# Siverteh/semantic-slam-master

Measured on AMD Instinct MI355X. Metric: frames/sec extract+match on TUM 640x480; match-index bit-exact vs CPU ref, higher is better.
Workload: dtype f32

## Files before the change

semantic-slam-master_amd/csrc/common.h:

```cpp
#pragma once

#include <hip/hip_runtime.h>
#include <stdint.h>

#include "../../include/sslam_hip.h"

typedef float f32x16 __attribute__((ext_vector_type(16)));
typedef float f32x4 __attribute__((ext_vector_type(4)));

extern long long g_sslam_launches;
static inline void sslam_count_launches(long long n) { __atomic_fetch_add(&g_sslam_launches, n, __ATOMIC_RELAXED); }

enum sslam_knob_id {
    KNOB_M1_VARIANT,
    KNOB_CONV_VARIANT,
    KNOB_CONV_LATENCY_ROWS,
    KNOB_CONV_LAT2_ROWS,
    KNOB_CONV_NO_HALO,
    KNOB_CONV_TAIL,
    KNOB_CONVBF_NO_HALO,
    KNOB_CONVBF_TAIL,
    KNOB_CONVBF_VARIANT,
    KNOB_VIT_NO_FUSED_MLP,
    KNOB_BN_FORM,
    KNOB_VIT_F32_NO_KEY_SPLIT,
    KNOB_RT_STOP,
    KNOB_REFINE_DISTINCT,
    KNOB_COUNT
};
#define SSLAM_KNOB_UNSET (-0x7fffffffffffffffLL - 1)
extern long long g_sslam_knob[KNOB_COUNT];
static inline long long sslam_knob(int id, long long dflt) { const long long v = g_sslam_knob[id]; return v == SSLAM_KNOB_UNSET ? dflt : v; }
static inline bool sslam_knob_set(int id) { return g_sslam_knob[id] != SSLAM_KNOB_UNSET; }

template <class... P>
static inline bool sslam_misaligned(unsigned a, P... p) {
    uintptr_t bits = 0;
    const uintptr_t each[] = {(uintptr_t)p...};
    for (const uintptr_t v : each) bits |= v;
    return (bits & (uintptr_t)(a - 1)) != 0;
}

#define SSLAM_CHECK_LAUNCH()                                   \
    do {                                                       \
        sslam_count_launches(1);                               \
        if (hipGetLastError() != hipSuccess) return SSLAM_E_LAUNCH; \
    } while (0)

__host__ __device__ inline int kp8(int k) { return (k & ~7) | ((k & 1) << 2) | ((k & 7) >> 1); }

__device__ __forceinline__ f32x16 mfma32(float a, float b, f32x16 c) {
    return __builtin_amdgcn_mfma_f32_32x32x2f32(a, b, c, 0, 0, 0);
}

__device__ __forceinline__ int crow(int r, int h) { return (r & 3) + 8 * (r >> 2) + 4 * h; }

__device__ __forceinline__ float bfly32(float v) {
    v = v + __shfl_xor(v, 16);
    v = v + __shfl_xor(v, 8);
    v = v + __shfl_xor(v, 4);
// ... 52 lines not shown
```

semantic-slam-master_amd/csrc/lib.hip:

```cpp
#include <stdlib.h>
#include <string.h>

#include "common.h"

long long g_sslam_launches = 0;
long long g_sslam_knob[KNOB_COUNT];

namespace {
long long g_knob_at_load[KNOB_COUNT];
const char *const kKnobNames[KNOB_COUNT] = {
    "SSLAM_M1_VARIANT",   "SSLAM_CONV_VARIANT",  "SSLAM_CONV_LATENCY_ROWS", "SSLAM_CONV_LAT2_ROWS",   "SSLAM_CONV_NO_HALO",
    "SSLAM_CONV_TAIL",    "SSLAM_CONVBF_NO_HALO", "SSLAM_CONVBF_TAIL",      "SSLAM_CONVBF_VARIANT",   "SSLAM_VIT_NO_FUSED_MLP",
    "SSLAM_BN_FORM",      "SSLAM_VIT_F32_NO_KEY_SPLIT", "SSLAM_RT_STOP",
    "SSLAM_REFINE_DISTINCT"};
struct KnobInit {
    KnobInit() {
        for (int i = 0; i < KNOB_COUNT; i++) {
            const char *e = getenv(kKnobNames[i]);
            g_sslam_knob[i] = g_knob_at_load[i] = e ? atoll(e) : SSLAM_KNOB_UNSET;
        }
    }
} g_knob_init;
}

extern "C" int sslam_version(void) { return 650; }
extern "C" const char *sslam_arch(void) { return "gfx950"; }
extern "C" long long sslam_launch_count(void) { return __atomic_load_n(&g_sslam_launches, __ATOMIC_RELAXED); }

extern "C" long long sslam_workspace_bytes(int n_frames, int G, int K, int n_pairs) {
    if (n_frames <= 0 || G <= 0 || K <= 0 || n_pairs < 0) return SSLAM_E_INVALID;
    const long long a = sslam_selector_saliency_workspace_bytes(n_frames, G);
    const long long b = n_pairs > 0 ? sslam_sim_argmax_workspace_bytes(K, n_pairs) : 0;
    const long long c = sslam_gather_refine_workspace_bytes(n_frames, K);
    const long long m = a > b ? (a > c ? a : c) : (b > c ? b : c);
    return (m + 255) & ~255LL;
}

extern "C" int sslam_test_set_knob(const char *name, long long value, int unset) {
    if (!name) return SSLAM_E_INVALID;
    for (int i = 0; i < KNOB_COUNT; i++)
        if (!strcmp(name, kKnobNames[i])) {
            g_sslam_knob[i] = unset ? g_knob_at_load[i] : value;
            return SSLAM_OK;
        }
    return SSLAM_E_INVALID;
}
```

semantic-slam-master_amd/csrc/selector.hip:

```cpp
#include <stdlib.h>

#include "common.h"

namespace {

constexpr int BK = 32;
constexpr int LDT = BK + 4;
constexpr int NCHUNK = SSLAM_C / BK;
constexpr int NSTAGE = 9 * NCHUNK;

template <int WM, int WN, int NI, bool BDIRECT, int MI = 2>
__global__ __launch_bounds__(512, (BDIRECT && WM == 2) ? 4 : 1) void selector_saliency_kernel(const float *__restrict__ feat, int n_rows, int G,
                                                                 const float *__restrict__ w1p,
                                                                 const float *__restrict__ b1,
                                                                 const float *__restrict__ w2,
                                                                 const float *__restrict__ b2, float *__restrict__ sal,
                                                                 int n_tiles) {
    static_assert(WM * WN == 8, "8 waves");
    static_assert(MI == 2 || (MI == 1 && NI == 1 && BDIRECT), "latency form: one 32 x 32 tile per wave");
    constexpr int BM = 32 * MI * WM;
    constexpr int HS = 32 * NI * WN;
    constexpr int NSLAB = HS / 64;
    constexpr int A_ITEMS = BM * 4 >= 512 ? BM * 4 / 512 : 1;
    constexpr bool A_PART = BM * 4 < 512;
// ... 171 lines not shown
            for (int e = 0; e < 16; e++) {
                const float h1 = acc[0][0][e] > 0.0f ? acc[0][0][e] : 0.0f;
                xch[(slab * 16 + e) * 64 + lane] = h1 * w2v;
            }
        }
        __syncthreads();
        if (!(wn & 1)) {
#pragma unroll
            for (int e = 0; e < 16; e++) {
                const float h0 = acc[0][0][e] > 0.0f ? acc[0][0][e] : 0.0f;
                const float q = h0 * w2v + xch[(slab * 16 + e) * 64 + lane];
                const float t = bfly32(q);
                if (r == 0) red[slab * BM + crow(e, h)] = t;
            }
        }
    }
    __syncthreads();
    for (int t = tid; t < BM; t += 512) {
        const long long m = m0 + t;
        if (m < n_rows) {
            float logit = b2[0];
#pragma unroll
            for (int s = 0; s < NSLAB; s++) logit = logit + red[s * BM + t];
            sal[m] = sslam_sigmoid(logit);
        }
    }
}
#undef LOAD_STAGE
#undef STORE_STAGE

constexpr int HIMG_ROWS = 256;
constexpr int HIMG_FLOATS = HIMG_ROWS * LDT;

template <bool SMALL>
__device__ __forceinline__ void halo_tile(float *hsmem, const float *__restrict__ feat, int n_rows, int G, const float *__restrict__ w1p,
                                          const float *__restrict__ b1, const float *__restrict__ w2, const float *__restrict__ b2,
                                          float *__restrict__ sal, const int m0, const int m_end) {
    constexpr int WN = SMALL ? 8 : 4, NI = SMALL ? 1 : 2, MI = SMALL ? 1 : 2, BM = 32 * MI * (8 / WN), HS = 256, NSLAB = 4;
    const int tid = threadIdx.x, lane = tid & 63, wave = tid >> 6, r = lane & 31, h = lane >> 5;
    const int wm = wave / WN, wn = wave % WN;
    const int cells = G * G, G1 = G + 1, P = (G + 2) * G1;
    auto padded = [&](int m) {
        const int f = m / cells, c = m - f * cells, y = c / G, x = c - y * G;
        return f * P + (y + 1) * G1 + x;
    };
    const int p_lo = padded(m0) - (G + 2);

    const __amdgpu_buffer_rsrc_t frs =
        __builtin_amdgcn_make_buffer_rsrc(const_cast<float *>(feat), 0, (int)((unsigned)n_rows * (SSLAM_C * 4u)), 0x00020000);
    const int kq = tid & 3;
    int a_voff[2];
#pragma unroll
    for (int i = 0; i < 2; i++) {
        const int pr = p_lo + (tid >> 2) + 128 * i;
        int off = -32;
        if (pr >= 0) {
            const int f = pr / P, q = pr - f * P, yy = q / G1, xx = q - yy * G1;
            const long long m = (long long)f * cells + (yy - 1) * G + xx;
            if (yy >= 1 && yy <= G && xx < G && m < n_rows) off = (int)((unsigned)m * (SSLAM_C * 4u) + kq * 32u);
        }
        a_voff[i] = off;
    }
    float4 ra_lo, ra_hi;
#define HL(I, C)                                                                                                   \
    {                                                                                                              \
        ra_lo = __builtin_bit_cast(float4, __builtin_amdgcn_raw_buffer_load_b128(frs, a_voff[I], (C) * (BK * 4), 0));      \
        ra_hi = __builtin_bit_cast(float4, __builtin_amdgcn_raw_buffer_load_b128(frs, a_voff[I], (C) * (BK * 4) + 16, 0)); \
    }
#define HS_(I, BUF)                                                                                                \
    {                                                                                                              \
        float4 ev, od;                                                                                             \
        kp8_split(ra_lo, ra_hi, ev, od);                                                                           \
        float *d = hsmem + (BUF) * HIMG_FLOATS + ((tid >> 2) + 128 * (I)) * LDT + kq * 8;                          \
        *reinterpret_cast<float4 *>(d) = ev;                                                                       \
        *reinterpret_cast<float4 *>(d + 4) = od;                                                                   \
    }

    int a_base[MI];
#pragma unroll
    for (int mi = 0; mi < MI; mi++) {
        const int m = min(m0 + wm * 32 * MI + mi * 32 + r, m_end - 1);
        a_base[mi] = (padded(m) - p_lo) * LDT + 4 * h;
    }

    f32x16 acc[MI][NI];
#pragma unroll
    for (int ni = 0; ni < NI; ni++) {
        const float bv = b1[wn * 32 * NI + ni * 32 + r];
#pragma unroll
        for (int mi = 0; mi < MI; mi++)
#pragma unroll
            for (int e = 0; e < 16; e++) acc[mi][ni][e] = bv;
    }
    const f32x4 *bsrc = reinterpret_cast<const f32x4 *>(w1p) + ((wn * 32 * NI + r) * 2 + h);
    const __amdgpu_buffer_rsrc_t wrs =
        __builtin_amdgcn_make_buffer_rsrc(const_cast<float *>(w1p), 0, 9 * SSLAM_C * HS * 4, 0x00020000);
    const int b_voff = ((wn * 32 * NI + r) * 2 + h) * 16;
    f32x4 bq[BK / 8][NI];
#pragma unroll
    for (int g = 0; g < BK / 8; g++)
#pragma unroll
        for (int ni = 0; ni < NI; ni++) bq[g][ni] = bsrc[((long long)g * HS + ni * 32) * 2];

    HL(0, 0);
    HS_(0, 0);
    HL(1, 0);
    HS_(1, 0);
    __syncthreads();
    int tap = 0, dy = -1, dx = -1, chunk = 0;
    for (int s = 0; s < NSTAGE; s++) {
        if (chunk + 1 < NCHUNK) {
            if (tap == 0) HL(0, chunk + 1);
            if (tap == 4) {
                HS_(0, (chunk + 1) & 1);
                HL(1, chunk + 1);
            }
        }
        const float *img = hsmem + (chunk & 1) * HIMG_FLOATS + (dy * G1 + dx) * LDT;
        const float *A0 = img + a_base[0], *A1 = img + a_base[MI - 1];
        __builtin_amdgcn_s_setprio(1);
#pragma unroll
        for (int g = 0; g < BK / 8; g++) {
            const f32x4 a0 = *reinterpret_cast<const f32x4 *>(A0 + 8 * g);
            f32x4 a1 = a0;
            if (MI == 2) a1 = *reinterpret_cast<const f32x4 *>(A1 + 8 * g);
            f32x4 b[NI];
#pragma unroll
            for (int ni = 0; ni < NI; ni++) b[ni] = bq[g][ni];
#pragma unroll
            for (int st = 0; st < 4; st++)
#pragma unroll
                for (int ni = 0; ni < NI; ni++) {
                    acc[0][ni] = mfma32(a0[st], b[ni][st], acc[0][ni]);
                    if (MI == 2) acc[MI - 1][ni] = mfma32(a1[st], b[ni][st], acc[MI - 1][ni]);
                }
            if (s + 1 < NSTAGE && (g == BK / 16 - 1 || g == BK / 8 - 1)) {
#pragma unroll
                for (int gg = g + 1 - BK / 16; gg <= g; gg++)
#pragma unroll
                    for (int ni = 0; ni < NI; ni++)
                        bq[gg][ni] = __builtin_bit_cast(f32x4, __builtin_amdgcn_raw_buffer_load_b128(
                                                            wrs, b_voff, (((s + 1) * (BK / 8) + gg) * HS + ni * 32) * 32, 0));
            }
            if (g == BK / 16 - 1) __builtin_amdgcn_sched_barrier(0);
        }
        __builtin_amdgcn_s_setprio(0);
        tap++; dx++;
        if (dx == 2) { dx = -1; dy++; }
        if (tap == 9) {
            if (chunk + 1 < NCHUNK) HS_(1, (chunk + 1) & 1);
            __syncthreads();
            tap = 0; dy = -1; chunk++;
        }
    }
#undef HL
#undef HS_
    __syncthreads();
    float *red = hsmem;
    if (!SMALL) {
#pragma unroll
        for (int sl = 0; sl < NI / 2; sl++) {
            const int slab = wn * (NI / 2) + sl;
            const float w2a = w2[slab * 64 + r], w2b = w2[slab * 64 + 32 + r];
#pragma unroll
            for (int mi = 0; mi < MI; mi++)
#pragma unroll
                for (int e = 0; e < 16; e++) {
                    const float h0 = acc[mi][2 * sl][e] > 0.0f ? acc[mi][2 * sl][e] : 0.0f;
                    const float h1 = acc[mi][NI > 1 ? 2 * sl + 1 : 0][e] > 0.0f ? acc[mi][NI > 1 ? 2 * sl + 1 : 0][e] : 0.0f;
                    const float q = h0 * w2a + h1 * w2b;
                    const float t = bfly32(q);
                    if (r == 0) red[slab * BM + wm * 64 + mi * 32 + crow(e, h)] = t;
                }
        }
    } else {
        float *xch = hsmem + NSLAB * BM;
        const int slab = wn >> 1;
        const float w2v = w2[wn * 32 + r];
        if (wn & 1) {
#pragma unroll
            for (int e = 0; e < 16; e++) {
                const float h1 = acc[0][0][e] > 0.0f ? acc[0][0][e] : 0.0f;
                xch[(slab * 16 + e) * 64 + lane] = h1 * w2v;
            }
        }
        __syncthreads();
        if (!(wn & 1)) {
#pragma unroll
            for (int e = 0; e < 16; e++) {
                const float h0 = acc[0][0][e] > 0.0f ? acc[0][0][e] : 0.0f;
                const float q = h0 * w2v + xch[(slab * 16 + e) * 64 + lane];
                const float t = bfly32(q);
                if (r == 0) red[slab * BM + crow(e, h)] = t;
            }
        }
    }
    __syncthreads();
    for (int t = tid; t < BM; t += 512) {
        const long long m = (long long)m0 + t;
        if (m < m_end) {
            float logit = b2[0];
#pragma unroll
            for (int sb = 0; sb < NSLAB; sb++) logit = logit + red[sb * BM + t];
            sal[m] = sslam_sigmoid(logit);
        }
    }
}

__global__ __launch_bounds__(512, 4) void selector_saliency_halo_kernel(const float *__restrict__ feat, int n_rows, int G,
                                                                         const float *__restrict__ w1p, const float *__restrict__ b1,
                                                                         const float *__restrict__ w2, const float *__restrict__ b2,
                                                                         float *__restrict__ sal, int n_big) {
    extern __shared__ __attribute__((aligned(16))) float hsmem[];
    const int b = blockIdx.x;
    if (b < n_big) {
        const int q = n_big / 8, rem = n_big % 8, x = b % 8;
        const int tile = (x < rem ? x * (q + 1) : rem * (q + 1) + (x - rem) * q) + b / 8;
        halo_tile<false>(hsmem, feat, n_rows, G, w1p, b1, w2, b2, sal, tile * 128, n_rows);
    } else {
        halo_tile<true>(hsmem, feat, n_rows, G, w1p, b1, w2, b2, sal, n_big * 128 + (b - n_big) * 32, n_rows);
    }
}

__global__ __launch_bounds__(512, 4) void selector_saliency_halo_frames_kernel(const float *__restrict__ feat, int n_rows, int G,
                                                                                const float *__restrict__ w1p, const float *__restrict__ b1,
                                                                                const float *__restrict__ w2, const float *__restrict__ b2,
                                                                                float *__restrict__ sal, int n_big, int n_quarter, int tb, int ts) {
    extern __shared__ __attribute__((aligned(16))) float hsmem[];
    const int b = blockIdx.x, cells = G * G;
    if (b < n_big) {
        const int q = n_big / 8, rem = n_big % 8, x = b % 8;
        const int tile = (x < rem ? x * (q + 1) : rem * (q + 1) + (x - rem) * q) + b / 8;
        const int f = tile / tb, j = tile - f * tb;
        halo_tile<false>(hsmem, feat, n_rows, G, w1p, b1, w2, b2, sal, f * cells + j * 128, (f + 1) * cells);
    } else if (b < n_big + n_quarter) {
        const int u = b - n_big, tile = n_big + (u >> 2);
        const int f = tile / tb, j = tile - f * tb;
        halo_tile<true>(hsmem, feat, n_rows, G, w1p, b1, w2, b2, sal, f * cells + j * 128 + (u & 3) * 32, (f + 1) * cells);
    } else {
        const int u = b - n_big - n_quarter, f = u / ts, j = u - f * ts;
        halo_tile<true>(hsmem, feat, n_rows, G, w1p, b1, w2, b2, sal, f * cells + tb * 128 + j * 32, (f + 1) * cells);
    }
}

template <int NP>
__global__ __launch_bounds__(256) void selector_saliency_lat2_kernel(const float *__restrict__ feat, int n_rows, int G,
                                                                      const float *__restrict__ w1p, const float *__restrict__ b1,
                                                                      const float *__restrict__ w2, float *__restrict__ part) {
    constexpr int HS = 256, BM = 32;
    constexpr int IMG_FLOATS = NP * 64 * LDT;
    extern __shared__ __attribute__((aligned(16))) float hsmem[];
    const int tid = threadIdx.x, lane = tid & 63, wn = tid >> 6, r = lane & 31, h = lane >> 5;
    const int half = blockIdx.x & 1, tile = blockIdx.x >> 1;
    const int col0 = half * 128 + wn * 32;
    const int cells = G * G, G1 = G + 1, P = (G + 2) * G1;
    const int m0 = tile * BM;
    auto padded = [&](int m) {
        const int f = m / cells, c = m - f * cells, y = c / G, x = c - y * G;
        return f * P + (y + 1) * G1 + x;
    };
    const int p_lo = padded(m0) - (G + 2);
    const __amdgpu_buffer_rsrc_t frs =
        __builtin_amdgcn_make_buffer_rsrc(const_cast<float *>(feat), 0, (int)((unsigned)n_rows * (SSLAM_C * 4u)), 0x00020000);
    const int kq = tid & 3;
    int a_voff[NP];
#pragma unroll
    for (int i = 0; i < NP; i++) {
        const int pr = p_lo + (tid >> 2) + 64 * i;
        int off = -32;
        if (pr >= 0) {
            const int f = pr / P, q = pr - f * P, yy = q / G1, xx = q - yy * G1;
            const long long m = (long long)f * cells + (yy - 1) * G + xx;
            if (yy >= 1 && yy <= G && xx < G && m < n_rows) off = (int)((unsigned)m * (SSLAM_C * 4u) + kq * 32u);
        }
        a_voff[i] = off;
// ... 131 lines not shown
    thread_local int c_G = 0, c_val = 0;
    if (G == c_G) return c_val;
    const int cells = G * G, G1 = G + 1;
    auto padded = [&](int c) { const int y = c / G, x = c - y * G; return (y + 1) * G1 + x; };
    int worst = 0;
    const int tb = cells / 128;
    for (int t = 0; t < tb; t++) {
        const int need = padded(t * 128 + 127) - padded(t * 128) + 2 * (G + 2) + 1;
        worst = need > worst ? need : worst;
    }
    for (int c0 = tb * 128; c0 < cells; c0 += 32) {
        const int c1 = c0 + 31 < cells - 1 ? c0 + 31 : cells - 1;
        const int need = padded(c1) - padded(c0) + 2 * (G + 2) + 1;
        worst = need > worst ? need : worst;
    }
    c_G = G, c_val = worst;
    return worst;
}

template <int WM, int WN, int NI, bool BD, int MI = 2>
void launch(const float *feat, long long rows, int G, const float *w1p, const float *b1, const float *w2, const float *b2,
            float *sal, hipStream_t st) {
    constexpr int BM = 32 * MI * WM;
    const int n_tiles = (int)((rows + BM - 1) / BM);
    hipLaunchKernelGGL((selector_saliency_kernel<WM, WN, NI, BD, MI>), dim3(n_tiles), dim3(512), 0, st, feat, (int)rows, G, w1p, b1,
                       w2, b2, sal, n_tiles);
}

}

static const long long LAT2_DEFAULT_ROWS = 32 * 25 * 6;
static const long long LAT_DEFAULT_ROWS = 128 * 1800;

extern "C" long long sslam_selector_saliency_workspace_bytes(int n_frames, int G) {
    if (n_frames <= 0 || G <= 0) return SSLAM_E_INVALID;
    const long long rows = (long long)n_frames * G * G;
    return rows <= sslam_knob(KNOB_CONV_LAT2_ROWS, LAT2_DEFAULT_ROWS) ? rows * 16 : 0;
}

extern "C" int sslam_selector_saliency_ws(const float *feat, int n_frames, int G, const float *w1_packed, const float *b1,
                                          const float *w2, const float *b2, int hs, float *sal, void *workspace,
                                          long long workspace_bytes, void *stream) {
    if (!feat || !w1_packed || !b1 || !w2 || !b2 || !sal || n_frames <= 0 || G <= 0) return SSLAM_E_INVALID;
    if (((uintptr_t)feat | (uintptr_t)w1_packed | (uintptr_t)workspace) & 15) return SSLAM_E_INVALID;
    if (sslam_misaligned(4, b1, w2, b2, sal)) return SSLAM_E_INVALID;
    const long long rows = (long long)n_frames * G * G;
    if (rows * (long long)(SSLAM_C * 4) > 0xffffffffLL) return SSLAM_E_UNSUPPORTED;
    hipStream_t st = (hipStream_t)stream;
    const int variant = (int)sslam_knob(KNOB_CONV_VARIANT, 2);
    const long long lat_rows = sslam_knob(KNOB_CONV_LATENCY_ROWS, LAT_DEFAULT_ROWS);
    const long long lat2_rows = sslam_knob(KNOB_CONV_LAT2_ROWS, LAT2_DEFAULT_ROWS);
    if (hs == 256 && rows <= lat2_rows && rows <= lat_rows && workspace && workspace_bytes >= rows * 16) {
        const int np = (halo_rows32(G, rows) + 63) / 64;
        if (np <= 6) {
            float *part = (float *)workspace;
            const int n_tiles = (int)((rows + 31) / 32);
#define LAT2(NP_)                                                                                                              \
    hipLaunchKernelGGL((selector_saliency_lat2_kernel<NP_>), dim3(2 * n_tiles), dim3(256), 2 * NP_ * 64 * LDT * sizeof(float), st, feat, \
                       (int)rows, G, w1_packed, b1, w2, part)
            switch (np) {
                case 6: LAT2(6); break;
                case 5: LAT2(5); break;
                case 4: LAT2(4); break;
                case 3: LAT2(3); break;
                default: LAT2(2); break;
            }
#undef LAT2
            SSLAM_CHECK_LAUNCH();
            hipLaunchKernelGGL(saliency_finish_kernel, dim3((unsigned)((rows + 255) / 256)), dim3(256), 0, st, part, b2, (int)rows, sal);
            SSLAM_CHECK_LAUNCH();
            return SSLAM_OK;
        }
    }
    if (hs == 256 && rows <= lat_rows) {
        launch<1, 8, 1, true, 1>(feat, rows, G, w1_packed, b1, w2, b2, sal, st);
    } else if (hs == 256 && variant == 2 && !sslam_knob(KNOB_CONV_NO_HALO, 0) && halo_rows128(G, rows) <= HIMG_ROWS) {
        const int n_tiles = (int)((rows + 127) / 128);
        const int round = (int)sslam_knob(KNOB_CONV_TAIL, 512);
        const int n_big = round > 0 && n_tiles > round ? n_tiles / round * round : n_tiles;
        const int n_small = n_big < n_tiles ? (int)((rows - (long long)n_big * 128 + 31) / 32) : 0;
        hipLaunchKernelGGL(selector_saliency_halo_kernel, dim3(n_big + n_small), dim3(512), 2 * HIMG_FLOATS * sizeof(float), st, feat, (int)rows, G,
                           w1_packed, b1, w2, b2, sal, n_big);
    } else if (hs == 256 && variant == 2 && !sslam_knob(KNOB_CONV_NO_HALO, 0) && G * G >= 128 && halo_rows_frame(G) <= HIMG_ROWS) {
        const int cells = G * G, tb = cells / 128, ts = (cells - tb * 128 + 31) / 32;
        const long long nb = (long long)n_frames * tb;
        const int round = (int)sslam_knob(KNOB_CONV_TAIL, 512);
        const long long n_big = round > 0 && nb > round ? nb / round * round : nb;
        const long long n_quarter = (nb - n_big) * 4, n_small = (long long)n_frames * ts;
        hipLaunchKernelGGL(selector_saliency_halo_frames_kernel, dim3((unsigned)(n_big + n_quarter + n_small)), dim3(512),
                           2 * HIMG_FLOATS * sizeof(float), st, feat, (int)rows, G, w1_packed, b1, w2, b2, sal, (int)n_big, (int)n_quarter, tb, ts);
    } else if (hs == 256) {
        switch (variant) {
            case 0: launch<2, 4, 2, false>(feat, rows, G, w1_packed, b1, w2, b2, sal, st); break;
            case 1: launch<4, 2, 4, false>(feat, rows, G, w1_packed, b1, w2, b2, sal, st); break;
            case 3: launch<4, 2, 4, true>(feat, rows, G, w1_packed, b1, w2, b2, sal, st); break;
            default: launch<2, 4, 2, true>(feat, rows, G, w1_packed, b1, w2, b2, sal, st); break;
        }
    } else if (hs == 128) {
        if (variant >= 2)
            launch<4, 2, 2, true>(feat, rows, G, w1_packed, b1, w2, b2, sal, st);
        else
            launch<4, 2, 2, false>(feat, rows, G, w1_packed, b1, w2, b2, sal, st);
    } else {
        return SSLAM_E_UNSUPPORTED;
    }
    SSLAM_CHECK_LAUNCH();
    return SSLAM_OK;
}
// ... 19 lines not shown
```

semantic-slam-master_amd/sslam_amd/lib.py:

```python
from __future__ import annotations

import ctypes as C
import os
import subprocess

import numpy as np
import torch

_PKG = os.path.dirname(os.path.dirname(os.path.abspath(__file__)))
CSRC = os.path.join(_PKG, "csrc")
SO_PATH = os.path.join(CSRC, "libsslam_hip.so")

OK, E_INVALID, E_UNSUPPORTED, E_LAUNCH = 0, -1, -2, -3
_ERR = {E_INVALID: "invalid argument", E_UNSUPPORTED: "unsupported shape", E_LAUNCH: "kernel launch failed"}

C_FEAT, HID, D_OUT = 384, 384, 128
WIDTHS = (128, 256)
MAX_TAPS = 32


class SslamHipError(RuntimeError):
    pass


# ... 52 lines not shown
    "sslam_row_lse", "sslam_row_lse_pairs", "sslam_edge_pool", "sslam_val_frame_stats", "sslam_val_pair_stats",
    "sslam_val_pair_stats_pairs",
    "sslam_refiner_layout_d", "sslam_refiner_pack_host_d", "sslam_refine_d", "sslam_gather_refine_d", "sslam_gather_refine_ws_d",
    "sslam_sim_argmax_d", "sslam_sim_argmax_ws_d", "sslam_sim_argmax_pairs_d", "sslam_sim_argmax_rows_d",
    "sslam_sim_argmax_rows_pairs_d", "sslam_row_lse_d", "sslam_row_lse_pairs_d", "sslam_val_frame_stats_d",
    "sslam_match_rank", "sslam_pose_nn_pairs", "sslam_match_score_pairs",
    "sslam_keypoint_depth", "sslam_pose_depth_nn_pairs", "sslam_match_score_known_pairs",
    "sslam_pose_ransac_pairs", "sslam_pose_refine_pairs",
]


def lib():
    global _lib
    if _lib is None:
        if not os.path.exists(SO_PATH):
            raise SslamHipError(f"{SO_PATH} is missing: run `python -c 'import __graft_entry__ as g; g.build()'` "
                                f"(or `make -C {CSRC}`); this package has no non-HIP execution path")
        L = C.CDLL(SO_PATH)
        L.sslam_arch.restype = C.c_char_p
        L.sslam_launch_count.restype = C.c_longlong
        p, i, ll, f, d = C.c_void_p, C.c_int, C.c_longlong, C.c_float, C.c_double
        L.sslam_pack_conv3x3_host.argtypes = [p, i, p]
        L.sslam_pack_linear_host.argtypes = [p, i, i, p]
        L.sslam_resample_table_host.argtypes = [i, i, i, p, p, i]
        L.sslam_preprocess_u8.argtypes = [p, i, i, i, i, p, p, i, p, p, i, p, p]
        L.sslam_preprocess_u8_patches.argtypes = [p, i, i, i, i, p, p, i, p, p, i, p, p]
        L.sslam_bn_tokens.argtypes = [p, i, i, i, i, p, p, p, p, i, f, p, p, p, p]
        L.sslam_selector_saliency.argtypes = [p, i, i, p, p, p, p, i, p, p]
        L.sslam_selector_saliency_ws.argtypes = [p, i, i, p, p, p, p, i, p, p, ll, p]
        for fn, at in ((L.sslam_workspace_bytes, [i, i, i, i]), (L.sslam_selector_saliency_workspace_bytes, [i, i]),
                       (L.sslam_sim_argmax_workspace_bytes, [i, i]), (L.sslam_gather_refine_workspace_bytes, [i, i])):
            fn.restype, fn.argtypes = ll, at
        L.sslam_test_set_knob.argtypes = [C.c_char_p, ll, i]
        L.sslam_select_keypoints.argtypes = [p, i, i, i, i, d, p, p, p, p, p, p]
        L.sslam_gather.argtypes = [p, i, i, p, i, p, p]
        L.sslam_refiner_layout.argtypes = [i, C.POINTER(RefinerLayout)]
        L.sslam_refiner_pack_host.argtypes = [p, i, p]
        L.sslam_refine.argtypes = [p, ll, p, i, p, p]
        L.sslam_gather_refine.argtypes = [p, i, i, p, i, p, i, p, p]
        L.sslam_gather_refine_ws.argtypes = [p, i, i, p, i, p, i, p, p, ll, p]
        L.sslam_keypoint_intensity.argtypes = [p, i, i, i, i, p, p, i, p, p, i, p, i, p, p]
        L.sslam_sim_argmax.argtypes = [p, ll, i, p, ll, i, i, p, p, p, p, p, p]
        L.sslam_sim_argmax_ws.argtypes = [p, ll, i, p, ll, i, i, p, p, p, p, p, p, ll, p]
        L.sslam_match_finalize.argtypes = [p, p, p, i, i, i, p, ll, p, ll, p, p, f, f, f, f, f, p, p, p, p]
        L.sslam_sim_argmax_pairs.argtypes = [p, ll, i, i, p, p, i, p, p, p, p, p, p, ll, p]
        L.sslam_match_finalize_pairs.argtypes = [p, p, p, i, i, p, p, i, p, ll, p, f, f, f, f, f, p, p, p, p]
        L.sslam_match_finalize_rule.argtypes = [p, p, p, p, i, i, i, i, f, p, p, p, p]
        L.sslam_match_finalize_rule_pairs.argtypes = [p, p, p, p, i, i, p, p, i, i, f, p, p, p, p]
        L.sslam_match_rank.argtypes = [p, p, p, i, i, i, i, p, p, p, p, p]
        L.sslam_pose_nn_pairs.argtypes = [p, i, i, i, i, p, p, i, p, d, p, p, p, p, p, p]
        L.sslam_match_score_pairs.argtypes = [p, p, p, p, p, i, i, p, p, p, p, p]
        L.sslam_keypoint_depth.argtypes = [p, i, i, i, p, i, d, d, p, p]
        L.sslam_pose_depth_nn_pairs.argtypes = [p, p, i, i, i, i, p, p, i, p] + [d] * 10 + [p, p, p, p, p, p, p]
        L.sslam_match_score_known_pairs.argtypes = [p, p, p, p, p, i, i, p, p, p, p, p, p]
        L.sslam_pose_ransac_pairs.argtypes = [p, p, i, i, p, p, i, p, p, i] + [d] * 10 + [i, C.c_uint64] + [p] * 7 + [p]
        L.sslam_pose_refine_pairs.argtypes = [p, p, i, i, p, p, i, p, p, i] + [d] * 10 + [p, d, i] + [p] * 12 + [p]
        L.sslam_sim_argmax_rows.argtypes = [p, ll, i, p, ll, i, i, p, p, p, p]
        L.sslam_sim_argmax_rows_pairs.argtypes = [p, ll, i, i, p, p, i, p, p, p, p]
        L.sslam_row_lse.argtypes = [p, ll, i, p, ll, i, i, p, f, p, p, p, p]
        L.sslam_row_lse_pairs.argtypes = [p, ll, i, i, p, p, i, p, f, p, p, p, p]
        L.sslam_edge_pool.argtypes = [p, i, i, p, p, p]
        L.sslam_val_frame_stats.argtypes = [p, p, p, p, i, i, i, p, p, p, p]
        L.sslam_val_pair_stats.argtypes = [p, p, i, p, p, p, p, p, i, i, i, f, p, p, p]
        L.sslam_val_pair_stats_pairs.argtypes = [p, i, i, p, p, p, p, p, p, p, i, i, f, p, p, p]
        L.sslam_refiner_layout_d.argtypes = [i, i, C.POINTER(RefinerLayout)]
        L.sslam_refiner_pack_host_d.argtypes = [p, i, i, p]
# ... 245 lines not shown
    w = np.ascontiguousarray(w, np.float32)
    hs = w.shape[0]
    assert w.shape == (hs, C_FEAT, 3, 3)
    out = np.empty(9 * C_FEAT * hs, np.uint16)
    _check(lib().sslam_pack_conv3x3_bf16_host(w.ctypes.data, hs, out.ctypes.data), "pack_conv3x3_bf16")
    return out


def to_bf16(x, out=None):
    x = x.contiguous()
    if out is None:
        out = torch.empty(x.shape, dtype=torch.bfloat16, device=x.device)
    _run("f32_to_bf16", lib().sslam_f32_to_bf16, (x, out,),
         _dp(x), _dp(out), x.numel())
    return out


def selector_saliency_bf16(feat_bf16, w1p_bf16, b1, w2, b2, hs, out=None):
    n, g = feat_bf16.shape[0], feat_bf16.shape[1]
    if out is None:
        out = torch.empty((n, g, g), dtype=torch.float32, device=feat_bf16.device)
    _run("selector_saliency_bf16", lib().sslam_selector_saliency_bf16, (feat_bf16, w1p_bf16, b1, w2, b2, out,),
         _dp(feat_bf16), n, g, _dp(w1p_bf16), _dp(b1), _dp(w2), _dp(b2), hs, _dp(out))
    return out


def selector_bf16_halo_groups(n_frames: int, G: int, hs: int = 256) -> int:
    np_ = int(lib().sslam_selector_bf16_halo_groups(n_frames, G, hs))
    if np_ < 0:
        _check(np_, "selector_bf16_halo_groups")
    return np_


def select_keypoints(sal, K, radius=2, pct=0.5, want_idx=True, want_pixel=True, out=None):
    n, g = sal.shape[0], sal.shape[1]
    dev = sal.device
    if out is not None:
        kp, sc, idx, px, st = out
    else:
        kp = torch.empty((n, K, 2), dtype=torch.float32, device=dev)
        sc = torch.empty((n, K), dtype=torch.float32, device=dev)
        idx = torch.empty((n, K), dtype=torch.int32, device=dev) if want_idx else None
        px = torch.empty((n, K, 2), dtype=torch.float32, device=dev) if want_pixel else None
        st = torch.empty((n,), dtype=torch.int32, device=dev)
    _run("select_keypoints", lib().sslam_select_keypoints, (sal, kp, sc, idx, px, st,),
         _dp(sal), n, g, K, radius, C.c_double(pct), _dp(kp), _dp(sc), _dp(idx), _dp(px),
                                        _dp(st))
    return kp, sc, idx, px, st


def gather(feat, kp, out=None):
    n, g = feat.shape[0], feat.shape[1]
    K = kp.shape[1]
    if out is None:
        out = torch.empty((n, K, C_FEAT), dtype=torch.float32, device=feat.device)
    _run("gather", lib().sslam_gather, (feat, kp, out,),
         _dp(feat), n, g, _dp(kp), K, _dp(out))
    return out


def refine(x, packed, n_blocks, out=None):
    rows = x.numel() // C_FEAT
    d = packed_refiner_width(packed, n_blocks)
    if out is None:
        out = torch.empty(x.shape[:-1] + (d,), dtype=torch.float32, device=x.device)
    elif out.numel() != rows * d:
# ... 988 lines not shown
```

Before: 59080.

## Split selector 3x3 conv into interior and border-class tiles with tap skipping

Adds a border-aware saliency conv kernel that tiles interior cells in 128-row blocks and handles the top/bottom/left/right edges and the interior remainder as separate small tiles. The edge tiles use compact halo images and skip the MFMA work and weight prefetch for taps that fall outside the grid. The shared halo compute is factored into a halo_core template. The goal is to cut the padded-halo waste and the zero-tap MFMA work on edge cells, at the cost of extra index arithmetic, more tile kinds, and a more complex launch plan.

```diff
diff --git a/semantic-slam-master_amd/csrc/common.h b/semantic-slam-master_amd/csrc/common.h
--- a/semantic-slam-master_amd/csrc/common.h
+++ b/semantic-slam-master_amd/csrc/common.h
@@ -26,6 +26,7 @@
     KNOB_VIT_F32_NO_KEY_SPLIT,
     KNOB_RT_STOP,
     KNOB_REFINE_DISTINCT,
+    KNOB_CONV_BORDER,
     KNOB_COUNT
 };
 #define SSLAM_KNOB_UNSET (-0x7fffffffffffffffLL - 1)
diff --git a/semantic-slam-master_amd/csrc/lib.hip b/semantic-slam-master_amd/csrc/lib.hip
--- a/semantic-slam-master_amd/csrc/lib.hip
+++ b/semantic-slam-master_amd/csrc/lib.hip
@@ -12,7 +12,7 @@
     "SSLAM_M1_VARIANT",   "SSLAM_CONV_VARIANT",  "SSLAM_CONV_LATENCY_ROWS", "SSLAM_CONV_LAT2_ROWS",   "SSLAM_CONV_NO_HALO",
     "SSLAM_CONV_TAIL",    "SSLAM_CONVBF_NO_HALO", "SSLAM_CONVBF_TAIL",      "SSLAM_CONVBF_VARIANT",   "SSLAM_VIT_NO_FUSED_MLP",
     "SSLAM_BN_FORM",      "SSLAM_VIT_F32_NO_KEY_SPLIT", "SSLAM_RT_STOP",
-    "SSLAM_REFINE_DISTINCT"};
+    "SSLAM_REFINE_DISTINCT", "SSLAM_CONV_BORDER"};
 struct KnobInit {
     KnobInit() {
         for (int i = 0; i < KNOB_COUNT; i++) {
diff --git a/semantic-slam-master_amd/csrc/selector.hip b/semantic-slam-master_amd/csrc/selector.hip
--- a/semantic-slam-master_amd/csrc/selector.hip
+++ b/semantic-slam-master_amd/csrc/selector.hip
@@ -227,35 +227,17 @@
 constexpr int HIMG_ROWS = 256;
 constexpr int HIMG_FLOATS = HIMG_ROWS * LDT;
 
-template <bool SMALL>
-__device__ __forceinline__ void halo_tile(float *hsmem, const float *__restrict__ feat, int n_rows, int G, const float *__restrict__ w1p,
+template <bool SMALL, bool SKIPS, class SalIndex>
+__device__ __forceinline__ void halo_core(float *hsmem, const float *__restrict__ feat, int n_rows, const float *__restrict__ w1p,
                                           const float *__restrict__ b1, const float *__restrict__ w2, const float *__restrict__ b2,
-                                          float *__restrict__ sal, const int m0, const int m_end) {
+                                          float *__restrict__ sal, const int (&a_voff)[2], const int (&a_base)[SMALL ? 1 : 2], const int tap_stride,
+                                          const int skip, SalIndex sal_index) {
     constexpr int WN = SMALL ? 8 : 4, NI = SMALL ? 1 : 2, MI = SMALL ? 1 : 2, BM = 32 * MI * (8 / WN), HS = 256, NSLAB = 4;
     const int tid = threadIdx.x, lane = tid & 63, wave = tid >> 6, r = lane & 31, h = lane >> 5;
     const int wm = wave / WN, wn = wave % WN;
-    const int cells = G * G, G1 = G + 1, P = (G + 2) * G1;
-    auto padded = [&](int m) {
-        const int f = m / cells, c = m - f * cells, y = c / G, x = c - y * G;
-        return f * P + (y + 1) * G1 + x;
-    };
-    const int p_lo = padded(m0) - (G + 2);
-
     const __amdgpu_buffer_rsrc_t frs =
         __builtin_amdgcn_make_buffer_rsrc(const_cast<float *>(feat), 0, (int)((unsigned)n_rows * (SSLAM_C * 4u)), 0x00020000);
     const int kq = tid & 3;
-    int a_voff[2];
-#pragma unroll
-    for (int i = 0; i < 2; i++) {
-        const int pr = p_lo + (tid >> 2) + 128 * i;
-        int off = -32;
-        if (pr >= 0) {
-            const int f = pr / P, q = pr - f * P, yy = q / G1, xx = q - yy * G1;
-            const long long m = (long long)f * cells + (yy - 1) * G + xx;
-            if (yy >= 1 && yy <= G && xx < G && m < n_rows) off = (int)((unsigned)m * (SSLAM_C * 4u) + kq * 32u);
-        }
-        a_voff[i] = off;
-    }
     float4 ra_lo, ra_hi;
 #define HL(I, C)                                                                                                   \
     {                                                                                                              \
@@ -271,13 +253,6 @@
         *reinterpret_cast<float4 *>(d + 4) = od;                                                                   \
     }
 
-    int a_base[MI];
-#pragma unroll
-    for (int mi = 0; mi < MI; mi++) {
-        const int m = min(m0 + wm * 32 * MI + mi * 32 + r, m_end - 1);
-        a_base[mi] = (padded(m) - p_lo) * LDT + 4 * h;
-    }
-
     f32x16 acc[MI][NI];
 #pragma unroll
     for (int ni = 0; ni < NI; ni++) {
@@ -292,10 +267,13 @@
         __builtin_amdgcn_make_buffer_rsrc(const_cast<float *>(w1p), 0, 9 * SSLAM_C * HS * 4, 0x00020000);
     const int b_voff = ((wn * 32 * NI + r) * 2 + h) * 16;
     f32x4 bq[BK / 8][NI];
+    int s_first = 0;
+    if (SKIPS)
+        while ((skip >> s_first) & 1) s_first++;
 #pragma unroll
     for (int g = 0; g < BK / 8; g++)
 #pragma unroll
-        for (int ni = 0; ni < NI; ni++) bq[g][ni] = bsrc[((long long)g * HS + ni * 32) * 2];
+        for (int ni = 0; ni < NI; ni++) bq[g][ni] = bsrc[((long long)(s_first * (BK / 8) + g) * HS + ni * 32) * 2];
 
     HL(0, 0);
     HS_(0, 0);
@@ -311,35 +289,45 @@
                 HL(1, chunk + 1);
             }
         }
-        const float *img = hsmem + (chunk & 1) * HIMG_FLOATS + (dy * G1 + dx) * LDT;
-        const float *A0 = img + a_base[0], *A1 = img + a_base[MI - 1];
-        __builtin_amdgcn_s_setprio(1);
-#pragma unroll
-        for (int g = 0; g < BK / 8; g++) {
-            const f32x4 a0 = *reinterpret_cast<const f32x4 *>(A0 + 8 * g);
-            f32x4 a1 = a0;
-            if (MI == 2) a1 = *reinterpret_cast<const f32x4 *>(A1 + 8 * g);
-            f32x4 b[NI];
-#pragma unroll
-            for (int ni = 0; ni < NI; ni++) b[ni] = bq[g][ni];
-#pragma unroll
-            for (int st = 0; st < 4; st++)
-#pragma unroll
-                for (int ni = 0; ni < NI; ni++) {
-                    acc[0][ni] = mfma32(a0[st], b[ni][st], acc[0][ni]);
-                    if (MI == 2) acc[MI - 1][ni] = mfma32(a1[st], b[ni][st], acc[MI - 1][ni]);
+        if (!SKIPS || !((skip >> tap) & 1)) {
+            int s_next = s + 1;
+            if (SKIPS) {
+                int t = tap + 1 == 9 ? 0 : tap + 1;
+                while ((skip >> t) & 1) {
+                    s_next++;
+                    t = t + 1 == 9 ? 0 : t + 1;
                 }
-            if (s + 1 < NSTAGE && (g == BK / 16 - 1 || g == BK / 8 - 1)) {
-#pragma unroll
-                for (int gg = g + 1 - BK / 16; gg <= g; gg++)
-#pragma unroll
-                    for (int ni = 0; ni < NI; ni++)
-                        bq[gg][ni] = __builtin_bit_cast(f32x4, __builtin_amdgcn_raw_buffer_load_b128(
-                                                            wrs, b_voff, (((s + 1) * (BK / 8) + gg) * HS + ni * 32) * 32, 0));
             }
-            if (g == BK / 16 - 1) __builtin_amdgcn_sched_barrier(0);
-        }
-        __builtin_amdgcn_s_setprio(0);
+            const float *img = hsmem + (chunk & 1) * HIMG_FLOATS + (dy * tap_stride + dx) * LDT;
+            const float *A0 = img + a_base[0], *A1 = img + a_base[MI - 1];
+            __builtin_amdgcn_s_setprio(1);
+#pragma unroll
+            for (int g = 0; g < BK / 8; g++) {
+                const f32x4 a0 = *reinterpret_cast<const f32x4 *>(A0 + 8 * g);
+                f32x4 a1 = a0;
+                if (MI == 2) a1 = *reinterpret_cast<const f32x4 *>(A1 + 8 * g);
+                f32x4 b[NI];
+#pragma unroll
+                for (int ni = 0; ni < NI; ni++) b[ni] = bq[g][ni];
+#pragma unroll
+                for (int st = 0; st < 4; st++)
+#pragma unroll
+                    for (int ni = 0; ni < NI; ni++) {
+                        acc[0][ni] = mfma32(a0[st], b[ni][st], acc[0][ni]);
+                        if (MI == 2) acc[MI - 1][ni] = mfma32(a1[st], b[ni][st], acc[MI - 1][ni]);
+                    }
+                if (s_next < NSTAGE && (g == BK / 16 - 1 || g == BK / 8 - 1)) {
+#pragma unroll
+                    for (int gg = g + 1 - BK / 16; gg <= g; gg++)
+#pragma unroll
+                        for (int ni = 0; ni < NI; ni++)
+                            bq[gg][ni] = __builtin_bit_cast(f32x4, __builtin_amdgcn_raw_buffer_load_b128(
+                                                                wrs, b_voff, ((s_next * (BK / 8) + gg) * HS + ni * 32) * 32, 0));
+                }
+                if (g == BK / 16 - 1) __builtin_amdgcn_sched_barrier(0);
+            }
+            __builtin_amdgcn_s_setprio(0);
+        }
         tap++; dx++;
         if (dx == 2) { dx = -1; dy++; }
         if (tap == 9) {
@@ -392,14 +380,51 @@
     }
     __syncthreads();
     for (int t = tid; t < BM; t += 512) {
-        const long long m = (long long)m0 + t;
-        if (m < m_end) {
+        const long long m = sal_index(t);
+        if (m >= 0) {
             float logit = b2[0];
 #pragma unroll
             for (int sb = 0; sb < NSLAB; sb++) logit = logit + red[sb * BM + t];
             sal[m] = sslam_sigmoid(logit);
         }
     }
+}
+
+template <bool SMALL>
+__device__ __forceinline__ void halo_tile(float *hsmem, const float *__restrict__ feat, int n_rows, int G, const float *__restrict__ w1p,
+                                          const float *__restrict__ b1, const float *__restrict__ w2, const float *__restrict__ b2,
+                                          float *__restrict__ sal, const int m0, const int m_end) {
+    constexpr int WN = SMALL ? 8 : 4, MI = SMALL ? 1 : 2;
+    const int tid = threadIdx.x, lane = tid & 63, wave = tid >> 6, r = lane & 31, h = lane >> 5;
+    const int wm = wave / WN;
+    const int cells = G * G, G1 = G + 1, P = (G + 2) * G1;
+    auto padded = [&](int m) {
+        const int f = m / cells, c = m - f * cells, y = c / G, x = c - y * G;
+        return f * P + (y + 1) * G1 + x;
+    };
+    const int p_lo = padded(m0) - (G + 2);
+
+    const int kq = tid & 3;
+    int a_voff[2];
+#pragma unroll
+    for (int i = 0; i < 2; i++) {
+        const int pr = p_lo + (tid >> 2) + 128 * i;
+        int off = -32;
+        if (pr >= 0) {
+            const int f = pr / P, q = pr - f * P, yy = q / G1, xx = q - yy * G1;
+            const long long m = (long long)f * cells + (yy - 1) * G + xx;
+            if (yy >= 1 && yy <= G && xx < G && m < n_rows) off = (int)((unsigned)m * (SSLAM_C * 4u) + kq * 32u);
+        }
+        a_voff[i] = off;
+    }
+    int a_base[MI];
+#pragma unroll
+    for (int mi = 0; mi < MI; mi++) {
+        const int m = min(m0 + wm * 32 * MI + mi * 32 + r, m_end - 1);
+        a_base[mi] = (padded(m) - p_lo) * LDT + 4 * h;
+    }
+    halo_core<SMALL, false>(hsmem, feat, n_rows, w1p, b1, w2, b2, sal, a_voff, a_base, G1, 0,
+                            [=](int t) { return m0 + t < m_end ? (long long)m0 + t : -1LL; });
 }
 
 __global__ __launch_bounds__(512, 4) void selector_saliency_halo_kernel(const float *__restrict__ feat, int n_rows, int G,
@@ -436,6 +461,162 @@
         const int u = b - n_big - n_quarter, f = u / ts, j = u - f * ts;
         halo_tile<true>(hsmem, feat, n_rows, G, w1p, b1, w2, b2, sal, f * cells + tb * 128 + j * 32, (f + 1) * cells);
     }
+}
+
+enum { BT_BIG, BT_TOP, BT_BOTTOM, BT_LEFT, BT_RIGHT, BT_REST, BT_KINDS };
+
+struct BorderGeom {
+    int f0, nf;
+    int seg, lead;
+    int dy_rows;
+    int c_lo;
+    int skip;
+    int valid;
+    int rows;
+};
+
+__host__ __device__ inline int border_per_frame(int G, int kind) {
+    const int in = (G - 2) * (G - 2);
+    return kind == BT_TOP || kind == BT_BOTTOM ? G : kind == BT_LEFT || kind == BT_RIGHT ? G - 2 : kind == BT_REST ? in % 128 : 128;
+}
+
+__host__ __device__ inline int border_interior_cell(int G, int i) { return (1 + i / (G - 2)) * G + 1 + i % (G - 2); }
+
+__host__ __device__ inline bool border_cell(int G, int F, int kind, int tile, int slot, int &f, int &c) {
+    if (kind == BT_BIG) {
+        const int nb = (G - 2) * (G - 2) / 128;
+        f = tile / nb;
+        c = border_interior_cell(G, (tile - f * nb) * 128 + slot);
+        return true;
+    }
+    const int per = border_per_frame(G, kind);
+    const long long p = (long long)tile * 32 + slot;
+    if (p >= (long long)F * per) return false;
+    f = (int)(p / per);
+    const int j = (int)(p - (long long)f * per);
+    c = kind == BT_TOP ? j : kind == BT_BOTTOM ? (G - 1) * G + j : kind == BT_LEFT ? (1 + j) * G : kind == BT_RIGHT ? (1 + j) * G + G - 1
+                       : border_interior_cell(G, (G - 2) * (G - 2) / 128 * 128 + j);
+    return true;
+}
+
+__host__ __device__ inline BorderGeom border_geom(int G, int F, int kind, int tile) {
+    BorderGeom g;
+    g.lead = 0, g.skip = 0, g.c_lo = 0;
+    if (kind == BT_BIG) {
+        int f, c0, c1;
+        border_cell(G, F, kind, tile, 0, f, c0);
+        border_cell(G, F, kind, tile, 127, f, c1);
+        g.f0 = f, g.nf = 1, g.valid = 128;
+        g.c_lo = c0 - G - 1, g.seg = c1 - c0 + 2 * (G + 1) + 1, g.dy_rows = G;
+    } else {
+        const int per = border_per_frame(G, kind);
+        const long long p0 = (long long)tile * 32, last = (long long)F * per - 1, p1 = p0 + 31 < last ? p0 + 31 : last;
+        g.f0 = (int)(p0 / per), g.nf = (int)(p1 / per) - g.f0 + 1, g.valid = (int)(p1 - p0) + 1;
+        if (kind == BT_REST) {
+            g.c_lo = border_interior_cell(G, (G - 2) * (G - 2) / 128 * 128) - G - 1;
+            g.seg = G * G - g.c_lo, g.dy_rows = G;
+        } else if (kind == BT_TOP || kind == BT_BOTTOM) {
+            g.seg = 2 * (G + 1), g.lead = 1, g.dy_rows = G + 1;
+            g.skip = kind == BT_TOP ? 0x007 : 0x1c0;
+        } else {
+            g.seg = 2 * G, g.dy_rows = 2;
+            g.skip = kind == BT_LEFT ? 0x049 : 0x124;
+        }
+    }
+    g.rows = g.lead + g.nf * g.seg;
+    return g;
+}
+
+__host__ __device__ inline int border_image_row(const BorderGeom &g, int G, int kind, int f, int c) {
+    const int y = c / G, x = c - y * G;
+    const int local = kind == BT_BIG || kind == BT_REST ? c - g.c_lo
+                      : kind == BT_TOP                   ? x
+                      : kind == BT_BOTTOM                ? G + 1 + x
+                      : kind == BT_LEFT                  ? 2 * y
+                                                         : 2 * y + 1;
+    return g.lead + (f - g.f0) * g.seg + local;
+}
+
+__host__ __device__ inline long long border_row_cell(const BorderGeom &g, int G, int kind, int q) {
+    q -= g.lead;
+    if (q < 0 || q >= g.nf * g.seg) return -1;
+    const int j = q / g.seg, rr = q - j * g.seg;
+    int c;
+    if (kind == BT_BIG || kind == BT_REST) {
+        c = g.c_lo + rr;
+    } else if (kind == BT_TOP || kind == BT_BOTTOM) {
+        const int yy = rr / (G + 1), xx = rr - yy * (G + 1);
+        if (xx == G) return -1;
+        c = ((kind == BT_TOP ? 0 : G - 2) + yy) * G + xx;
+    } else {
+        c = (rr >> 1) * G + (kind == BT_LEFT ? 0 : G - 2) + (rr & 1);
+    }
+    return (long long)(g.f0 + j) * G * G + c;
+}
+
+template <bool SMALL>
+__device__ __forceinline__ void border_tile(float *hsmem, const float *__restrict__ feat, int n_rows, int G, int F, const float *__restrict__ w1p,
+                                            const float *__restrict__ b1, const float *__restrict__ w2, const float *__restrict__ b2,
+                                            float *__restrict__ sal, const int kind, const int tile) {
+    constexpr int WN = SMALL ? 8 : 4, MI = SMALL ? 1 : 2;
+    const int tid = threadIdx.x, lane = tid & 63, wave = tid >> 6, r = lane & 31, h = lane >> 5;
+    const int wm = wave / WN, kq = tid & 3, cells = G * G;
+    const BorderGeom g = border_geom(G, F, kind, tile);
+    int a_voff[2];
+#pragma unroll
+    for (int i = 0; i < 2; i++) {
+        const long long m = border_row_cell(g, G, kind, (tid >> 2) + 128 * i);
+        a_voff[i] = m >= 0 ? (int)((unsigned)m * (SSLAM_C * 4u) + kq * 32u) : -32;
+    }
+    int a_base[MI];
+#pragma unroll
+    for (int mi = 0; mi < MI; mi++) {
+        int f, c;
+        border_cell(G, F, kind, tile, min(wm * 32 * MI + mi * 32 + r, g.valid - 1), f, c);
+        a_base[mi] = border_image_row(g, G, kind, f, c) * LDT + 4 * h;
+    }
+    halo_core<SMALL, SMALL>(hsmem, feat, n_rows, w1p, b1, w2, b2, sal, a_voff, a_base, g.dy_rows, g.skip, [=](int t) {
+        int f, c;
+        return border_cell(G, F, kind, tile, t, f, c) ? (long long)f * cells + c : -1LL;
+    });
+}
+
+struct BorderGrid {
+    int n_big, end[5];
+};
+
+__global__ __launch_bounds__(512, 4) void selector_saliency_border_kernel(const float *__restrict__ feat, int n_rows, int G, int F,
+                                                                          const float *__restrict__ w1p, const float *__restrict__ b1,
+                                                                          const float *__restrict__ w2, const float *__restrict__ b2,
+                                                                          float *__restrict__ sal, BorderGrid gr) {
+    extern __shared__ __attribute__((aligned(16))) float hsmem[];
+    const int b = blockIdx.x;
+    if (b < gr.n_big) {
+        const int q = gr.n_big / 8, rem = gr.n_big % 8, x = b % 8;
+        const int tile = (x < rem ? x * (q + 1) : rem * (q + 1) + (x - rem) * q) + b / 8;
+        border_tile<false>(hsmem, feat, n_rows, G, F, w1p, b1, w2, b2, sal, BT_BIG, tile);
+    } else {
+        int k = 0, start = gr.n_big;
+        while (k < 4 && b >= gr.end[k]) start = gr.end[k++];
+        border_tile<true>(hsmem, feat, n_rows, G, F, w1p, b1, w2, b2, sal, k == 0 ? BT_REST : k, b - start);
+    }
+}
+
+bool border_plan(int F, int G, long long tiles[BT_KINDS], int max_rows[BT_KINDS]) {
+    for (int k = 0; k < BT_KINDS; k++) tiles[k] = 0, max_rows[k] = 0;
+    if (F <= 0 || G < 3 || (G - 2) * (G - 2) < 128) return false;
+    bool fits = true;
+    for (int k = 0; k < BT_KINDS; k++) {
+        const int per = border_per_frame(G, k);
+        tiles[k] = k == BT_BIG ? (long long)F * ((G - 2) * (G - 2) / 128) : ((long long)F * per + 31) / 32;
+        const long long period = k == BT_BIG ? (G - 2) * (G - 2) / 128 : per, scan = tiles[k] < period ? tiles[k] : period;
+        for (long long t = 0; t < scan; t++) {
+            const int rows = border_geom(G, F, k, (int)t).rows;
+            max_rows[k] = rows > max_rows[k] ? rows : max_rows[k];
+        }
+        fits = fits && max_rows[k] <= HIMG_ROWS;
+    }
+    return fits && tiles[BT_BIG] + tiles[BT_REST] + 4 * tiles[BT_TOP] < 0x7fffffffLL;
 }
 
 template <int NP>
@@ -633,6 +814,58 @@
 static const long long LAT2_DEFAULT_ROWS = 32 * 25 * 6;
 static const long long LAT_DEFAULT_ROWS = 128 * 1800;
 
+extern "C" int sslami_selector_border_plan(int n_frames, int G, long long *tiles, int *max_rows) {
+    if (!tiles || !max_rows || n_frames <= 0 || G <= 0) return SSLAM_E_INVALID;
+    if ((long long)n_frames * G * G * (SSLAM_C * 4) > 0xffffffffLL) return SSLAM_E_UNSUPPORTED;
+    return border_plan(n_frames, G, tiles, max_rows) ? SSLAM_OK : SSLAM_E_UNSUPPORTED;
+}
+
+extern "C" int sslami_selector_border_owners(int n_frames, int G, int kind, long long tile0, int n, int *fyx) {
+    long long tiles[BT_KINDS];
+    int rows[BT_KINDS];
+    if (!fyx || kind < 0 || kind >= BT_KINDS || tile0 < 0 || n < 0) return SSLAM_E_INVALID;
+    const int rc = sslami_selector_border_plan(n_frames, G, tiles, rows);
+    if (rc != SSLAM_OK) return rc;
+    if (tile0 + n > tiles[kind]) return SSLAM_E_INVALID;
+    const int slots = kind == BT_BIG ? 128 : 32;
+    for (long long t = 0; t < n; t++)
+        for (int s = 0; s < slots; s++) {
+            int f = -1, c = 0, *o = fyx + (t * slots + s) * 3;
+            const bool has = border_cell(G, n_frames, kind, (int)(tile0 + t), s, f, c);
+            o[0] = has ? f : -1, o[1] = has ? c / G : -1, o[2] = has ? c % G : -1;
+        }
+    return SSLAM_OK;
+}
+
+extern "C" long long sslami_selector_border_check(int n_frames, int G) {
+    long long tiles[BT_KINDS], bad = 0;
+    int rows[BT_KINDS];
+    const int rc = sslami_selector_border_plan(n_frames, G, tiles, rows);
+    if (rc != SSLAM_OK) return rc;
+    for (int kind = 0; kind < BT_KINDS; kind++)
+        for (long long t = 0; t < tiles[kind]; t++) {
+            const BorderGeom g = border_geom(G, n_frames, kind, (int)t);
+            for (int s = 0, f, c; s < (kind == BT_BIG ? 128 : 32); s++) {
+                if (!border_cell(G, n_frames, kind, (int)t, s, f, c)) {
+                    bad += s < g.valid;
+                    continue;
+                }
+                const int y = c / G, x = c % G, row = border_image_row(g, G, kind, f, c);
+                bad += s >= g.valid;
+                for (int tap = 0; tap < 9; tap++) {
+                    const int dy = tap / 3 - 1, dx = tap % 3 - 1, q = row + dy * g.dy_rows + dx;
+                    const bool in_grid = y + dy >= 0 && y + dy < G && x + dx >= 0 && x + dx < G;
+                    const long long want = in_grid ? ((long long)f * G + y + dy) * G + x + dx : -1;
+                    if ((g.skip >> tap) & 1)
+                        bad += in_grid;
+                    else
+                        bad += q < 0 || q >= HIMG_ROWS || border_row_cell(g, G, kind, q) != want;
+                }
+            }
+        }
+    return bad;
+}
+
 extern "C" long long sslam_selector_saliency_workspace_bytes(int n_frames, int G) {
     if (n_frames <= 0 || G <= 0) return SSLAM_E_INVALID;
     const long long rows = (long long)n_frames * G * G;
@@ -651,6 +884,8 @@
     const int variant = (int)sslam_knob(KNOB_CONV_VARIANT, 2);
     const long long lat_rows = sslam_knob(KNOB_CONV_LATENCY_ROWS, LAT_DEFAULT_ROWS);
     const long long lat2_rows = sslam_knob(KNOB_CONV_LAT2_ROWS, LAT2_DEFAULT_ROWS);
+    long long b_tiles[BT_KINDS];
+    int b_rows[BT_KINDS];
     if (hs == 256 && rows <= lat2_rows && rows <= lat_rows && workspace && workspace_bytes >= rows * 16) {
         const int np = (halo_rows32(G, rows) + 63) / 64;
         if (np <= 6) {
@@ -675,6 +910,15 @@
     }
     if (hs == 256 && rows <= lat_rows) {
         launch<1, 8, 1, true, 1>(feat, rows, G, w1_packed, b1, w2, b2, sal, st);
+    } else if (hs == 256 && variant == 2 && !sslam_knob(KNOB_CONV_NO_HALO, 0) && halo_rows128(G, rows) <= HIMG_ROWS &&
+               sslam_knob(KNOB_CONV_BORDER, 1) != 0 && border_plan(n_frames, G, b_tiles, b_rows)) {
+        BorderGrid gr;
+        gr.n_big = (int)b_tiles[BT_BIG];
+        const int order[5] = {BT_REST, BT_TOP, BT_BOTTOM, BT_LEFT, BT_RIGHT};
+        int end = gr.n_big;
+        for (int k = 0; k < 5; k++) gr.end[k] = end += (int)b_tiles[order[k]];
+        hipLaunchKernelGGL(selector_saliency_border_kernel, dim3((unsigned)end), dim3(512), 2 * HIMG_FLOATS * sizeof(float), st, feat, (int)rows, G,
+                           n_frames, w1_packed, b1, w2, b2, sal, gr);
     } else if (hs == 256 && variant == 2 && !sslam_knob(KNOB_CONV_NO_HALO, 0) && halo_rows128(G, rows) <= HIMG_ROWS) {
         const int n_tiles = (int)((rows + 127) / 128);
         const int round = (int)sslam_knob(KNOB_CONV_TAIL, 512);
diff --git a/semantic-slam-master_amd/sslam_amd/lib.py b/semantic-slam-master_amd/sslam_amd/lib.py
--- a/semantic-slam-master_amd/sslam_amd/lib.py
+++ b/semantic-slam-master_amd/sslam_amd/lib.py
@@ -108,6 +108,9 @@
                        (L.sslam_sim_argmax_workspace_bytes, [i, i]), (L.sslam_gather_refine_workspace_bytes, [i, i])):
             fn.restype, fn.argtypes = ll, at
         L.sslam_test_set_knob.argtypes = [C.c_char_p, ll, i]
+        L.sslami_selector_border_plan.argtypes = [i, i, p, p]
+        L.sslami_selector_border_owners.argtypes = [i, i, i, ll, i, p]
+        L.sslami_selector_border_check.restype, L.sslami_selector_border_check.argtypes = ll, [i, i]
         L.sslam_select_keypoints.argtypes = [p, i, i, i, i, d, p, p, p, p, p, p]
         L.sslam_gather.argtypes = [p, i, i, p, i, p, p]
         L.sslam_refiner_layout.argtypes = [i, C.POINTER(RefinerLayout)]
@@ -419,6 +422,33 @@
     return np_
 
 
+BORDER_KINDS = ("big", "top", "bottom", "left", "right", "rest")
+
+
+def selector_border_plan(n_frames: int, G: int):
+    tiles, rows = (C.c_longlong * 6)(), (C.c_int * 6)()
+    rc = lib().sslami_selector_border_plan(n_frames, G, tiles, rows)
+    if rc not in (OK, E_UNSUPPORTED):
+        _check(rc, "selector_border_plan")
+    return rc == OK, dict(zip(BORDER_KINDS, tiles)), dict(zip(BORDER_KINDS, rows))
+
+
+def selector_border_check(n_frames: int, G: int) -> int:
+    bad = int(lib().sslami_selector_border_check(n_frames, G))
+    if bad < 0:
+        _check(bad, "selector_border_check")
+    return bad
+
+
+def selector_border_owners(n_frames: int, G: int, kind: str) -> np.ndarray:
+    ok, tiles, _ = selector_border_plan(n_frames, G)
+    if not ok:
+        raise SslamHipError(f"selector_border_owners: the border-class tiling does not apply to G = {G}")
+    out = np.empty((tiles[kind], 128 if kind == "big" else 32, 3), np.int32)
+    _check(lib().sslami_selector_border_owners(n_frames, G, BORDER_KINDS.index(kind), 0, tiles[kind], out.ctypes.data), "selector_border_owners")
+    return out
+
+
 def select_keypoints(sal, K, radius=2, pct=0.5, want_idx=True, want_pixel=True, out=None):
     n, g = sal.shape[0], sal.shape[1]
     dev = sal.device
```

New measurement: 60020, median of 6. +1.6%, better.
